# stefanopini/simple-HRNet

Hardware: AMD Instinct MI355X
Metric: person-crops/sec HRNet-W48 384x288 (model forward + heat-map decode) (higher is better)
Workload: dtype bf16; 1 GPU; HRNet-W48 384x288, batch=256 random crops per GPU, bf16 MFMA (BASELINE configs[2]); global_batch=256, micro_batch=256, lanes_per_gpu=1, parallelism=dp1 (crop sharding, RCCL all-gather of keypoints), weights=random-init seeded (synth_state_dict seed 0), BN stats randomised, engine_switches=

## Files before the change

### simple-hrnet_amd/csrc/conv3x3_lds.inc

```
typedef __attribute__((ext_vector_type(8))) __bf16 bf16x8;
typedef __attribute__((ext_vector_type(8))) short s16x8;
typedef __attribute__((ext_vector_type(4))) short s16x4;
typedef __attribute__((ext_vector_type(4))) float f32x4;
#define GLOBAL_AS __attribute__((address_space(1)))
typedef const GLOBAL_AS unsigned short *gcu16;
typedef GLOBAL_AS unsigned short *gu16;

__device__ __forceinline__ float relu1(float x) {
    float r;
    asm("v_max_f32 %0, 0, %1" : "=v"(r) : "v"(x));
    return r;
}

__device__ __forceinline__ void glds16(const GLOBAL_AS void *gsrc, char *lds_wave_base) {
    __builtin_amdgcn_global_load_lds(gsrc,
                                     (__attribute__((address_space(3))) void *)lds_wave_base, 16, 0, 0);
}

template <int KS_, int NRB_, int DT_ = DT_BF16>
struct C3Cfg {
    static constexpr int KS = KS_, NRB = NRB_;
    static constexpr int DT = DT_;
    static constexpr int PARTS = KS == 48 ? 2 : 1;
    static constexpr int CPP = KS == 48 ? 7 : 9;
// ... 435 lines not shown
            pk[i][2 * j + 1] = ok ? hi : 0u;
        }
    }
    asm volatile("s_waitcnt lgkmcnt(0)" ::: "memory");
    __builtin_amdgcn_s_barrier();
#pragma unroll
    for (int i = 0; i < NF; ++i) {
        const int yr = (i == NF - 1 ? row_last : row_first + i * 16) + li;
        const unsigned ya = lds0 + 2 * BBF_W + yr * ROWB + g * 24;
#pragma unroll
        for (int v = 0; v < 3; ++v)
            asm volatile("ds_write_b64 %0, %1 offset:%2" ::"v"(ya), "v"(u32x2{pk[i][2 * v], pk[i][2 * v + 1]}), "i"(v * 8) : "memory");
    }
    asm volatile("s_waitcnt lgkmcnt(0)" ::: "memory");
    __builtin_amdgcn_s_barrier();
}

template <int DT>
__device__ __forceinline__ void bbf_run(const Conv3Problem &p, const int mt0, const int tiles_this_block, const int nb, char *smem) {
    constexpr int KS = 48, NRB = 3, ROWB = 96, NCH = 14, BM = 512, MR = 4, NT = 512;
    typedef __attribute__((ext_vector_type(2))) unsigned u32x2;
    typedef __attribute__((ext_vector_type(4))) unsigned u32x4;
    const int tid = threadIdx.x, lane = tid & 63;
    const int wave = __builtin_amdgcn_readfirstlane(tid >> 6);
    const int li = lane & 15, g = lane >> 4;
    const int m = nb * p.hpwp;
    const int mtiles = (m + BM - 1) / BM;
    int ntile = mtiles - mt0;
    if (ntile > tiles_this_block) ntile = tiles_this_block;
    if (ntile <= 0) return;
    const int halo = p.wp + 1;
    const int xrows = BM + 4 * halo, yrows = BM + 2 * halo;
    const int xunits = xrows * 6;
    const int nfr = (yrows + 15) >> 4, base = nfr >> 3, extra = nfr & 7;
    const int cnt = base + (wave < extra ? 1 : 0);
    const int f0 = wave * base + (wave < extra ? wave : extra);
    const int row_first = f0 * 16;
    int row_last = (f0 + cnt - 1) * 16;
    if (row_last > yrows - 16) row_last = yrows - 16;
    const gcu16 in = (gcu16)p.in;
    const gu16 out = (gu16)p.out;
    const unsigned lds0 = (unsigned)(size_t)(__attribute__((address_space(3))) char *)smem;
    char *const xy = smem + 2 * BBF_W;

    int xoff[NCH];
#pragma unroll
    for (int c = 0; c < NCH; ++c) {
        int k0 = 32 * c + 8 * g;
        if (k0 >= 9 * KS) k0 = 0;
        const int tap = k0 / KS, ci = k0 - tap * KS;
        const int dh = tap / 3, dw = tap - 3 * dh;
        xoff[c] = (dh * p.wp + dw) * ROWB + (ci >> 3) * 16;
    }
    const int ch0 = g * 4 * NRB;
    const int bl = lane < KS ? lane : 0;
    const int bvec1 = __float_as_int(((const GLOBAL_AS float *)p.bias)[bl]);
    const int bvec2 = __float_as_int(((const GLOBAL_AS float *)p.bias2)[bl]);
    auto load_x = [&](int tt) {
        const long row0 = (long)(mt0 + tt) * BM - 2 * halo;
        const long lo = -(long)halo, hi = (long)m + halo + 511;
#pragma unroll
        for (int k = 0; k < BBF_XY / 16 / NT + 1; ++k) {
            if (k * NT + wave * 64 < xunits) {
                int u = k * NT + tid;
                asm volatile("" : "+v"(u));
                if (u >= xunits) u = xunits - 1;
                const int r = (int)(((unsigned)u * 43691u) >> 18);
                const int q8 = u - r * 6;
                long gr = row0 + r;
                gr = gr < lo ? lo : (gr > hi ? hi : gr);
                glds16((const GLOBAL_AS char *)(in + gr * KS + q8 * 8), xy + (k * NT + wave * 64) * 16);
            }
        }
    };
    constexpr int NXP = BBF_XY / 16 / NT + 1, NXR = 8;
    u32x4 xpre[NXR];
    const int r0u = (int)(((unsigned)tid * 43691u) >> 18), q0u = tid - r0u * 6;
    auto x_src = [&](int tt, int k) {
        const int row0 = (mt0 + tt) * BM - 2 * halo;
        int r = r0u, q8 = q0u;
        asm volatile("" : "+v"(r), "+v"(q8));
        r += 85 * k + (2 * k) / 6, q8 += (2 * k) % 6;
        if (q8 >= 6) q8 -= 6, ++r;
        if (r >= xrows) r = xrows - 1, q8 = 5;
        int gr = row0 + r;
        const int lo = -halo, hi = m + halo + 511;
        gr = gr < lo ? lo : (gr > hi ? hi : gr);
        return in + ((long)gr * KS + q8 * 8);
    };
    auto fetch_x = [&](int tt) {
#pragma unroll
        for (int k = 0; k < NXR; ++k) xpre[k] = *(const GLOBAL_AS u32x4 *)x_src(tt, k);
#pragma unroll
        for (int k = NXR; k < NXP; ++k)
            if (k * NT + wave * 64 < xunits) glds16((const GLOBAL_AS char *)x_src(tt, k), xy + (k * NT + wave * 64) * 16);
    };
    auto store_x = [&]() {
        const unsigned a0 = lds0 + 2 * BBF_W + tid * 16;
        asm volatile("s_waitcnt vmcnt(0)" ::: "memory");
#pragma unroll
        for (int k = 0; k < NXR; ++k)
            if (k * NT + wave * 64 < xunits)
                asm volatile("ds_write_b128 %0, %1 offset:%2" ::"v"(a0), "v"(xpre[k]), "i"(k * NT * 16) : "memory");
    };
    {
        const GLOBAL_AS char *w1 = (const GLOBAL_AS char *)p.w, *w2 = (const GLOBAL_AS char *)p.w2;
#pragma unroll
        for (int k = 0; k < (BBF_W / 16 + NT - 1) / NT; ++k) {
            const int u0 = k * NT + wave * 64;
            if (u0 < BBF_W / 16) {
                glds16(w1 + (size_t)(u0 + lane) * 16, smem + u0 * 16);
                glds16(w2 + (size_t)(u0 + lane) * 16, smem + BBF_W + u0 * 16);
            }
        }
        load_x(0);
    }
#ifdef HRN_C3_TIMING
    long long t_w = 0, t_c1 = 0, t_c1p = 0, t_c2 = 0, t_post = 0, t_epi = 0;
    C3_T(t_begin);
#endif
    for (int tt = 0; tt < ntile; ++tt) {
        C3_T(tA);
        if (tt == 0) asm volatile("s_waitcnt vmcnt(0)" ::: "memory");
        asm volatile("s_waitcnt lgkmcnt(0)" ::: "memory");
        __builtin_amdgcn_s_barrier();
        const long p0 = (long)(mt0 + tt) * BM;
        C3_T(tB);
        long long tC = 0;
        u32x2 rpre[MR][3];
        const unsigned res_a = lds0 + 2 * BBF_W + (wave * 16 * MR + li + 2 * halo) * ROWB + g * 24;
        if (cnt == 6)
            bbf_conv1<6, DT>(p, xoff, bvec1, lds0, row_first, row_last, p0 - halo, m, lane, res_a, rpre, tC);
        else if (cnt == 5)
            bbf_conv1<5, DT>(p, xoff, bvec1, lds0, row_first, row_last, p0 - halo, m, lane, res_a, rpre, tC);
        else
            bbf_conv1<4, DT>(p, xoff, bvec1, lds0, row_first, row_last, p0 - halo, m, lane, res_a, rpre, tC);
        C3_T(tD);
        if (tt + 1 < ntile) fetch_x(tt + 1);
        unsigned okbits2 = 0;
#pragma unroll
        for (int i = 0; i < MR; ++i) {
            const int q = (int)p0 + wave * 16 * MR + i * 16 + li;
            const int n_img = (int)(((unsigned long long)(unsigned)q * p.magic_hpwp) >> p.shift_hpwp);
            const int rem = q - n_img * p.hpwp;
            const int ho = (int)(((unsigned long long)(unsigned)rem * p.magic_wp) >> p.shift_wp);
            const int wo = rem - ho * p.wp;
            okbits2 |= ((q < m) && (ho < p.h) && (wo < p.wd)) ? 1u << i : 0u;
        }
        __builtin_amdgcn_sched_barrier(0);
        f32x4 acc[MR][NRB];
        {
            float bias2[4 * NRB];
#pragma unroll
            for (int c = 0; c < 4 * NRB; ++c) bias2[c] = __int_as_float(__builtin_amdgcn_ds_bpermute((ch0 + c) * 4, bvec2));
#pragma unroll
            for (int i = 0; i < MR; ++i)
#pragma unroll
                for (int j = 0; j < NRB; ++j) acc[i][j] = f32x4{bias2[j * 4], bias2[j * 4 + 1], bias2[j * 4 + 2], bias2[j * 4 + 3]};
        }
        {
            s16x8 wf[2][NRB], xf[2][MR];
            const unsigned wl_a = lds0 + BBF_W + lane * 16;
            unsigned sl_a = lds0 + 2 * BBF_W + (wave * 16 * MR + li) * ROWB;
            asm volatile("" : "+v"(sl_a));
#define BBF_READ2(SET, C)                                                                                         \
    {                                                                                                             \
        _Pragma("unroll") for (int j = 0; j < NRB; ++j)                                                           \
            asm volatile("ds_read_b128 %0, %1 offset:%2" : "=v"(wf[SET][j]) : "v"(wl_a), "i"(((C)*NRB + j) * 1024)); \
        const unsigned xa = sl_a + xoff[C];                                                                        \
        _Pragma("unroll") for (int i = 0; i < MR; ++i)                                                            \
            asm volatile("ds_read_b128 %0, %1 offset:%2" : "=v"(xf[SET][i]) : "v"(xa), "i"(i * 16 * ROWB));       \
    }
            BBF_READ2(0, 0)
#pragma unroll
            for (int c = 0; c < NCH; ++c) {
                const int cur = c & 1, nxt = cur ^ 1;
                if (c + 1 < NCH) {
                    BBF_READ2(nxt, c + 1)
                    asm volatile("s_waitcnt lgkmcnt(%0)" ::"i"(NRB + MR) : "memory");
                } else {
                    asm volatile("s_waitcnt lgkmcnt(0)" ::: "memory");
                }
                __builtin_amdgcn_sched_barrier(0);
#pragma unroll
                for (int i = 0; i < MR; ++i)
#pragma unroll
                    for (int j = 0; j < NRB; ++j)
                        acc[i][j] = H16<DT>::mma(wf[cur][j], xf[cur][i], acc[i][j]);
                __builtin_amdgcn_sched_barrier(0);
            }
#undef BBF_READ2
        }
        C3_T(tE);
        __builtin_amdgcn_s_barrier();
        if (tt + 1 < ntile) store_x();
        __builtin_amdgcn_sched_barrier(0);
        C3_T(tF);
#pragma unroll
        for (int i = 0; i < MR; ++i) {
            const int q = (int)p0 + wave * 16 * MR + i * 16 + li;
            const bool ok = (okbits2 >> i) & 1u;
            const size_t o = (size_t)q * KS + ch0;
            unsigned pk[2 * NRB];
#pragma unroll
            for (int j = 0; j < NRB; ++j) {
                const unsigned r01 = rpre[i][j][0], r23 = rpre[i][j][1];
                float v0 = acc[i][j][0] + H16<DT>::lo(r01);
                float v1 = acc[i][j][1] + H16<DT>::hi(r01);
                float v2 = acc[i][j][2] + H16<DT>::lo(r23);
                float v3 = acc[i][j][3] + H16<DT>::hi(r23);
                if (p.relu) v0 = relu1(v0), v1 = relu1(v1), v2 = relu1(v2), v3 = relu1(v3);
                const unsigned lo = H16<DT>::pk(v0, v1), hi = H16<DT>::pk(v2, v3);
                pk[2 * j] = ok ? lo : 0u;
                pk[2 * j + 1] = ok ? hi : 0u;
            }
            *(GLOBAL_AS u32x4 *)(out + o) = u32x4{pk[0], pk[1], pk[2], pk[3]};
            *(GLOBAL_AS u32x2 *)(out + o + 8) = u32x2{pk[4], pk[5]};
        }
#ifdef HRN_C3_TIMING
        C3_T(tG);
        t_w += tB - tA, t_c1 += tC - tB, t_c1p += tD - tC, t_c2 += tE - tD, t_post += tF - tE, t_epi += tG - tF;
#endif
    }
#ifdef HRN_C3_TIMING
    if (lane == 0 && g_c3_timing) {
        C3_T(t_end);
        long long *o = g_c3_timing + ((size_t)blockIdx.x * 8 + wave) * 8;
        o[0] = t_w, o[1] = t_c1, o[2] = t_c1p, o[3] = t_c2, o[4] = t_end - t_begin, o[5] = ntile, o[6] = 100 + cnt,
        o[7] = t_post | (t_epi << 32);
    }
#endif
}

#include "conv3x3_n96.inc"

template <int KS, int NRB, int DT>
__global__ __launch_bounds__(512, 2) void conv3x3_lds_kernel(const Conv3Problem *__restrict__ probs,
                                                             const int2 *__restrict__ blockmap, const int nb) {
    extern __shared__ __attribute__((aligned(16))) char smem[];
    using CFG = C3Cfg<KS, NRB, DT>;
#ifdef HRN_Q_TIMING
    struct Stamp {
        long long t0;
        __device__ Stamp() : t0((long long)__builtin_amdgcn_s_memrealtime()) {}
        __device__ ~Stamp() {
            if (g_q_timing && threadIdx.x == 0) {
                unsigned hw, xcc;
                asm volatile("s_getreg_b32 %0, hwreg(HW_REG_HW_ID)\n\ts_getreg_b32 %1, hwreg(HW_REG_XCC_ID)" : "=s"(hw), "=s"(xcc));
                const int seq = g_q_seq;
                long long *o = g_q_timing + ((size_t)(seq & (kQSlots - 1)) * kQBlocks + (blockIdx.x < kQBlocks ? blockIdx.x : kQBlocks - 1)) * 4;
                o[0] = t0, o[1] = (long long)gridDim.x | ((long long)seq << 32), o[2] = (long long)__builtin_amdgcn_s_memrealtime();
                o[3] = (long long)(((xcc & 15u) << 16) | (hw & 0xff00u));
            }
        }
    } stamp_;
#endif
    const int2 bm = blockmap[blockIdx.x];
    const Conv3Problem p = probs[bm.x & 0xff];
    const int nt = (bm.x >> 8) & 0xff, tiles = bm.x >> 16;
    const int mt0 = bm.y & 0x1fffffff;
    if constexpr (KS == 48 && NRB == 3) {
        if (bm.y & (1 << 29)) {
            bbf_run<DT>(p, mt0, tiles, nb, smem);
            return;
        }
        if (p.n96) {
            if (p.compact) {
                if (bm.y >> 30)
                    c3n_run<1, true, DT>(p, nt, mt0, tiles, nb, smem);
                else
                    c3n_run<4, true, DT>(p, nt, mt0, tiles, nb, smem);
                return;
            }
            if (bm.y >> 30)
                c3n_run<1, false, DT>(p, nt, mt0, tiles, nb, smem);
            else if (p.bm == 512)
                c3n_run<4, false, DT>(p, nt, mt0, tiles, nb, smem);
            else
                c3n_run<3, false, DT>(p, nt, mt0, tiles, nb, smem);
            return;
        }
    }
    if (bm.y >> 30) {
        conv3_run<CFG, 1>(p, nt, mt0, tiles, nb, smem);
    } else if constexpr (NRB == 4) {
        conv3_run<CFG, 3>(p, nt, mt0, tiles, nb, smem);
    } else {
        if (p.bm == 512)
            conv3_run<CFG, 4>(p, nt, mt0, tiles, nb, smem);
        else
            conv3_run<CFG, 3>(p, nt, mt0, tiles, nb, smem);
    }
}

template <int KS, int NRB, int DT>
static hipError_t launch_c3(const Conv3Problem *probs_dev, const int2 *blockmap_dev, int nblocks, int nb, hipStream_t s) {
// ... 27 lines not shown
```

### simple-hrnet_amd/csrc/ctx_memory.inc

```
    bool hip_ok(hipError_t e, const char *what) {
        if (e == hipSuccess) return true;
        err = std::string(what) + ": " + hipGetErrorString(e);
        return false;
    }

    bool allocate() {
        workspace_bytes = 0;
        for (auto &b : buffers) workspace_bytes += (int64_t)b.bytes;
        const int64_t small_crops = std::min<int64_t>(max_batch, (191 + head_slabs) / head_slabs);
        const int64_t part = std::max((int64_t)max_batch * joints * head_slabs, small_crops * joints * head_slabs_small);
        workspace_bytes += part * 8;
        if (plan_only) {
            fill_problems();
            index_s2groups();
            blob = (char *)calloc(1, (size_t)blob_bytes);
            return blob != nullptr;
        }
        if (!hip_ok(hipSetDevice(device), "hipSetDevice")) return false;
        for (auto &b : buffers) {
            if (!hip_ok(hipMalloc((void **)&b.dev, b.bytes), "hipMalloc(activation)")) return false;
            if (!hip_ok(hipMemset(b.dev, 0, b.bytes), "hipMemset(activation)")) return false;
        }
        if (!hip_ok(hipMalloc((void **)&blob, (size_t)blob_bytes), "hipMalloc(weights)")) return false;
        if (!hip_ok(hipMemset(blob, 0, (size_t)blob_bytes), "hipMemset(weights)")) return false;
// ... 18 lines not shown
    int group_blocks(const Conv3Group &g, int nb, std::vector<int2> *out, bool reverse, bool all_short = false,
                     std::vector<int> *tile_px_out = nullptr) const {
        struct Ent {
            double key;
            int2 v;
            int bm;
        };
        std::vector<Ent> ents;
        long one_per_block = 0;
        for (int ci : g.conv_idx) {
            const ConvOp &cv = convs[ci];
            if (skipped(cv, nb)) continue;
            const Tensor &to = tensors[cv.out_t];
            const int bmn = fused_now(cv, nb) ? 512 : conv3x3_lds_bm(cv.ks, cv.nr, to.wp);
            one_per_block += (long)((m_pixels(cv, to, nb) + bmn - 1) / bmn) * cv.ntiles;
        }
        const bool small = small_tiles && one_per_block < small_below;
        long small_blocks = 0;
        for (int ci : g.conv_idx) {
            const ConvOp &cv = convs[ci];
            if (skipped(cv, nb)) continue;
            small_blocks += (long)((m_pixels(cv, tensors[cv.out_t], nb) + 127) / 128) * cv.ntiles;
        }
        const bool keep_short_full = small && small_keep_above > 0 && small_blocks > small_keep_above;
        auto short_conv = [&](const ConvOp &cv) { return cv.ks != 16 && !cv.n96 && (cv.ks == 48 ? 2 : 1) * cv.slices <= 2; };
        auto small_conv = [&](const ConvOp &cv) {
            if (cv.ks == 16 && f32_small_slices > 0 && cv.slices >= f32_small_slices) return true;
            return small && !(keep_short_full && short_conv(cv));
        };
        auto tile_px = [&](const ConvOp &cv, const Tensor &to) {
            return fused_now(cv, nb) ? 512 : small_conv(cv) ? 128 : conv3x3_lds_bm(cv.ks, cv.nr, to.wp);
        };
        auto tiles_per_block = [&](const ConvOp &cv, int div) {
            return std::max(1, conv3_tiles_per_block(cv) / (fused_now(cv, nb) ? bbf_tpb_div : 1) / div);
        };
        auto count_blocks = [&](int div) {
            long total = 0;
            for (int ci : g.conv_idx) {
                const ConvOp &cv = convs[ci];
                if (skipped(cv, nb)) continue;
                const Tensor &to = tensors[cv.out_t];
                const int bm = tile_px(cv, to);
                const int mtiles = (int)((m_pixels(cv, to, nb) + bm - 1) / bm);
                const int tpb = tiles_per_block(cv, div);
                total += (long)((mtiles + tpb - 1) / tpb) * cv.ntiles;
            }
            return total;
        };
        int div = 1;
        while (div < 64 && count_blocks(div) < 512) div *= 2;
        int lf = all_short ? 1 : (int)std::min<long>(long_factor, count_blocks(div) / 768);
        if (lf < 1) lf = 1;
        for (size_t k = 0; k < g.conv_idx.size(); ++k) {
            const ConvOp &cv = convs[g.conv_idx[k]];
            if (skipped(cv, nb)) continue;
            const Tensor &to = tensors[cv.out_t];
            const int bm = tile_px(cv, to);
            const bool fused = fused_now(cv, nb);
            const int prob = fused ? g.fused_prob[k] : (int)k;
            const int mtiles = (int)((m_pixels(cv, to, nb) + bm - 1) / bm);
            const int tpb_short = tiles_per_block(cv, div);
            const int tpb_long = tpb_short * lf;
            const int long_tiles = ((int)(mtiles * long_share) / (8 * tpb_long)) * (8 * tpb_long);
            for (int phase = 0; phase < 2; ++phase) {
                const int tpb = phase == 0 ? tpb_long : tpb_short;
                const int first = phase == 0 ? 0 : long_tiles;
                const int count = phase == 0 ? long_tiles : mtiles - long_tiles;
                if (count <= 0) continue;
                const int mgroups = (count + tpb - 1) / tpb;
                const int total = mgroups * cv.ntiles;
                int seq = 0;
                for (int round = 0; round * 8 < mgroups; ++round)
                    for (int nt = 0; nt < cv.ntiles; ++nt)
                        for (int x = 0; x < 8; ++x) {
                            const int mg = round * 8 + x;
                            if (mg >= mgroups) continue;
                            const int i = seq++;
                            int tiles = count - mg * tpb;
                            if (tiles > tpb) tiles = tpb;
                            double key = (i + 0.5) / total;
                            if (block_order == 1)
                                key = -(double)tiles * (fused         ? 28000.0
                                                        : cv.ks == 16 ? cv.slices * (double)bm * 36.0 + 2000.0
                                                        : cv.n96      ? cv.slices * 3.0 * (bm == 512 ? 3900.0 : 3000.0) + (bm == 512 ? 7000.0 : 5000.0)
                                                                 : cv.slices * 2.0 * (bm == 512 ? 4300.0 : 3500.0) + (bm == 512 ? 5000.0 : 3000.0)) +
                                      1e-3 * key;
                            int mt0 = first + mg * tpb;
                            if (reverse) mt0 = mtiles - mt0 - tiles;
                            ents.push_back({key, int2{prob | (nt << 8) | (tiles << 16), mt0 | (fused ? 1 << 29 : small_conv(cv) ? 1 << 30 : 0)}, bm});
                        }
            }
        }
        std::stable_sort(ents.begin(), ents.end(), [](const Ent &a, const Ent &b) { return a.key < b.key; });
        if (tile_px_out) {
            tile_px_out->resize(ents.size());
            for (size_t i = 0; i < ents.size(); ++i) (*tile_px_out)[i] = ents[i].bm;
        }
        if (out) {
            out->resize(ents.size());
            for (size_t i = 0; i < ents.size(); ++i) (*out)[i] = ents[i].v;
        }
        return (int)ents.size();
    }

    const Tensor &grid_of(const ConvOp &cv) const { return tensors[cv.up ? cv.in_t : cv.out_t]; }

    ConvArgs conv_args(const ConvOp &cv, int nb, bool rev) const {
        const Tensor &ti = tensors[cv.in_t], &to = grid_of(cv);
        ConvArgs a;
        a.in = row0(cv.in_t), a.out = row0(cv.out_t);
        a.w = blob + cv.w_off, a.bias = (const float *)(blob + cv.b_off);
        a.res = cv.res_t >= 0 ? row0(cv.res_t) : nullptr;
        a.cin = cv.cin, a.cout = cv.cout;
        a.in_wp = ti.wp, a.in_hpwp = ti.hpwp;
        a.out_h = to.h, a.out_w = to.w, a.out_wp = to.wp, a.out_hpwp = to.hpwp;
        a.m = nb * to.hpwp;
        a.ksize = cv.k, a.stride = cv.stride, a.relu = cv.relu, a.kchunks = cv.kchunks;
        a.rev = rev;
// ... 240 lines not shown
        probs_host.assign(nprob, Conv3Problem{});
        std::vector<Conv3Problem> &hp = probs_host;
        for (auto &g : groups) {
            g.max_wp = 0;
            for (size_t k = 0; k < g.conv_idx.size(); ++k) {
                const ConvOp &cv = convs[g.conv_idx[k]];
                const Tensor &to = tensors[cv.out_t];
                Conv3Problem &q = hp[g.prob_first + k];
                q.in = row0(cv.in_t), q.out = row0(cv.out_t);
                q.w = blob + cv.w_off, q.bias = (const float *)(blob + cv.b_off);
                q.res = cv.res_t >= 0 ? row0(cv.res_t) : nullptr;
                q.cin = cv.cin, q.cout = cv.cout, q.h = to.h, q.wd = to.w, q.wp = to.wp, q.hpwp = to.hpwp;
                q.relu = cv.relu, q.slices = cv.slices, q.ntiles = cv.ntiles;
                q.w2 = nullptr, q.bias2 = nullptr;
                q.n96 = cv.n96 ? 1 : 0;
                q.compact = cv.compact ? 1 : 0, q.hw = to.h * to.w;
                q.slab_rows = q.slab_rows_small = 0;
                if (cv.compact) {
                    fast_div(q.hw, &q.magic_hw, &q.shift_hw);
                    fast_div(to.w, &q.magic_w, &q.shift_w);
                    q.slab_rows = compact_slab_rows(to.h, to.w, 512, max_batch), q.slab_rows_small = compact_slab_rows(to.h, to.w, 128, max_batch);
                }
                q.tiles_per_block = conv3_tiles_per_block(cv);
                q.bm = conv3x3_lds_bm(cv.ks, cv.nr, to.wp);
                fast_div(to.hpwp, &q.magic_hpwp, &q.shift_hpwp);
                fast_div(to.wp, &q.magic_wp, &q.shift_wp);
                if (to.wp > g.max_wp) g.max_wp = to.wp;
                if (cv.fuse_with >= 0) {
                    const ConvOp &c2 = convs[cv.fuse_with];
                    Conv3Problem &f = hp[g.prob_first + g.fused_prob[k]];
                    f = q;
                    f.out = row0(c2.out_t), f.relu = c2.relu, f.res = nullptr;
                    f.w2 = blob + c2.w_off, f.bias2 = (const float *)(blob + c2.b_off);
                }
            }
        }
        return nprob;
    }

    bool setup_groups() {
        const size_t nprob = fill_problems();
        if (!nprob) return true;
        std::vector<Conv3Problem> &hp = probs_host;
        for (auto &g : groups) {
            g.map_capacity = 64 + 4 * (int64_t)std::max(small_below, 256) + 1024;
            for (int ci : g.conv_idx) {
                const ConvOp &cv = convs[ci];
                const Tensor &to = tensors[cv.out_t];
                const int bm = f32_small_slices > 0 ? 128 : conv3x3_lds_bm(cv.ks, cv.nr, to.wp);
                g.map_capacity += (int64_t)((max_batch * to.hpwp + bm - 1) / bm) * cv.ntiles;
            }
            for (MapSlot &sl : g.slot) {
                if (!alloc_slot(sl, g.map_capacity, 0)) return false;
                workspace_bytes += g.map_capacity * (int64_t)sizeof(int2);
            }
        }
        if (!hip_ok(hipMalloc((void **)&probs_dev, nprob * sizeof(Conv3Problem)), "hipMalloc(problems)")) return false;
        return hip_ok(hipMemcpy(probs_dev, hp.data(), nprob * sizeof(Conv3Problem), hipMemcpyHostToDevice),
                      "hipMemcpy(problems)");
    }

    void free_all() {
        if (plan_only) {
            free(blob);
        } else {
            (void)hipSetDevice(device);
// ... 39 lines not shown
```

### simple-hrnet_amd/csrc/hrnet_mi355.cpp

```cpp
#include "../../include/hrnet_mi355.h"

#include <hip/hip_runtime.h>

#include <algorithm>
#include <cmath>
#include <cstdio>
#include <cstdlib>
#include <cstring>
#include <map>
#include <memory>
#include <string>
#include <vector>

#include "kernels.h"

namespace {
#include "ctx_types.h"
}

namespace {
thread_local std::string g_env_seen;
const char *env_sw(const char *name) {
    const char *v = hrn_env(name);
    if (v) {
// ... 27 lines not shown
        int conv3, conv1, ds;
        int conv2 = -1;
    };
    std::vector<Chain> chains;
    std::vector<TapPoint> taps;
    Conv3Problem *probs_dev = nullptr;
    std::vector<Op> ops;
    int stem_out_t = -1, head_in_t = -1;
    int64_t stem_w_off = 0, stem_b_off = 0, stem_wp_off = 0, head_w_off = 0, head_b_off = 0, head_wp_off = 0;

    int64_t blob_bytes = 0;
    char *blob = nullptr;
    bool weights_loaded = false;

    bool disable_lds = env_sw("HRN_DISABLE_LDS") != nullptr;
    bool disable_group = env_sw("HRN_DISABLE_GROUP") != nullptr;
    bool disable_dgroup = env_sw("HRN_DISABLE_DGROUP") != nullptr;
    bool disable_chain = env_sw("HRN_DISABLE_CHAIN") != nullptr;
    bool small_tiles = env_sw("HRN_SMALL_TILES") ? atoi(env_sw("HRN_SMALL_TILES")) != 0 : true;
    int small_below = env_sw("HRN_SMALL_BELOW") ? atoi(env_sw("HRN_SMALL_BELOW")) : 384;
    int small_keep_above = env_sw("HRN_SMALL_KEEP") ? atoi(env_sw("HRN_SMALL_KEEP")) : 300;
    bool disable_chain_ds = env_sw("HRN_DISABLE_CHAIN_DS") != nullptr;
    int pre_mode = env_sw("HRN_PRE_MODE") ? atoi(env_sw("HRN_PRE_MODE")) : 1;
    int chain_blocks = env_sw("HRN_CHAIN_BLOCKS") ? atoi(env_sw("HRN_CHAIN_BLOCKS")) : 512;
    bool disable_chain3 = env_sw("HRN_DISABLE_CHAIN3") != nullptr;
    bool direct_wlds = !(env_sw("HRN_DIRECT_WLDS") && atoi(env_sw("HRN_DIRECT_WLDS")) == 0);
    bool direct_xlds = !(env_sw("HRN_DIRECT_XLDS") && atoi(env_sw("HRN_DIRECT_XLDS")) == 0);
    bool conv_xl(const ConvOp &cv) const {
        return direct_xlds && direct_wlds && is16() && cv.k == 3 && cv.stride == 2 && cv.cin % 32 == 0 && !cv.up && cv.res_t < 0 && cv.nr == 6 &&
               cv.kchunks >= 4;
    }
    bool disable_bbf = env_sw("HRN_BBF") && atoi(env_sw("HRN_BBF")) == 0;
    int bbf_tpb_div = env_sw("HRN_BBF_TPB_DIV") ? std::max(1, atoi(env_sw("HRN_BBF_TPB_DIV"))) : 3;
    int bbf_min_tiles = env_sw("HRN_BBF_MIN_TILES") ? atoi(env_sw("HRN_BBF_MIN_TILES")) : 1100;
    int dgroup_nr_mode = env_sw("HRN_DGROUP_NR") ? atoi(env_sw("HRN_DGROUP_NR")) : 1;
    bool disable_lds32 = env_sw("HRN_DISABLE_LDS32") != nullptr;
    bool disable_n96 = env_sw("HRN_DISABLE_N96") != nullptr;
    bool disable_fgroup = env_sw("HRN_DISABLE_FGROUP") != nullptr;
    bool disable_f32lds = env_sw("HRN_DISABLE_F32LDS") != nullptr;
    int f32_small_slices = env_sw("HRN_F32_SMALL_SLICES") ? atoi(env_sw("HRN_F32_SMALL_SLICES")) : 0;
    std::vector<Conv3Problem> probs_host;
    bool disable_compact = env_sw("HRN_DISABLE_COMPACT") != nullptr;
    double compact_min_pad = env_sw("HRN_COMPACT_MIN_PAD") ? atof(env_sw("HRN_COMPACT_MIN_PAD")) : 0.08;
    bool disable_s2 = env_sw("HRN_DISABLE_S2") != nullptr;
    int s2_min_tiles = env_sw("HRN_S2_MIN_TILES") ? atoi(env_sw("HRN_S2_MIN_TILES")) : 256;
    int s2_target_blocks = env_sw("HRN_S2_BLOCKS") ? std::max(1, atoi(env_sw("HRN_S2_BLOCKS"))) : 256;
    bool disable_stem_mfma = env_sw("HRN_DISABLE_STEM_MFMA") != nullptr;
    bool disable_stem_fuse = env_sw("HRN_DISABLE_STEM_FUSE") != nullptr;
    bool stem_fuse = false;
    int stem_conv2_op = -1;
    S2Group stemf;
    bool disable_head_mfma = env_sw("HRN_DISABLE_HEAD_MFMA") != nullptr;
    bool direct_nr6 = env_sw("HRN_DIRECT_NR6") ? atoi(env_sw("HRN_DIRECT_NR6")) != 0 : true;
    int half_stages_per_block = env_sw("HRN_HALF_STAGES") ? atoi(env_sw("HRN_HALF_STAGES")) : 8;
    bool alternate = env_sw("HRN_ALTERNATE") ? atoi(env_sw("HRN_ALTERNATE")) != 0 : true;
    int block_order = env_sw("HRN_BLOCK_ORDER") ? atoi(env_sw("HRN_BLOCK_ORDER")) : 1;
    int long_factor = env_sw("HRN_LONG_FACTOR") ? atoi(env_sw("HRN_LONG_FACTOR")) : 4;
    double long_share = env_sw("HRN_LONG_SHARE") ? atof(env_sw("HRN_LONG_SHARE")) : 0.85;
    int head_slabs = 1, head_slab_px = 1024;
    static constexpr int kHeadSlabPxSmall = 256;
    int head_slabs_small = 1;
    int head_px_for(int nb) const { return (long)nb * head_slabs >= 192 ? head_slab_px : kHeadSlabPxSmall; }
    int head_slabs_for(int nb) const { return (long)nb * head_slabs >= 192 ? head_slabs : head_slabs_small; }
    float *part_val = nullptr;
    int *part_idx = nullptr;
    unsigned char *pre_tmp = nullptr;
// ... 645 lines not shown
```

### simple-hrnet_amd/csrc/kernels.h

```cpp
#pragma once
#include <hip/hip_runtime.h>
#include <stdint.h>

#include <atomic>
#include <cstdlib>
#include <cstring>

namespace hrn {

inline hipError_t set_dynamic_lds(const void *func, int bytes, std::atomic<unsigned long long> &done) {
    int dev = 0;
    hipError_t e = hipGetDevice(&dev);
    if (e != hipSuccess) return e;
    const unsigned long long bit = 1ull << (dev & 63);
    if (done.load(std::memory_order_acquire) & bit) return hipSuccess;
    e = hipFuncSetAttribute(func, hipFuncAttributeMaxDynamicSharedMemorySize, bytes);
    if (e == hipSuccess) done.fetch_or(bit, std::memory_order_release);
    return e;
}

inline const char *hrn_env(const char *name) {
    static const bool debug = [] {
        const char *v = getenv("HRN_DEBUG_ENV");
        return v && *v && strcmp(v, "0") != 0;
// ... 10 lines not shown
    const float *bias;
    const void *res;
    int cin, cout;
    int in_wp, in_hpwp;
    int out_h, out_w, out_wp, out_hpwp;
    int m;
    int ksize, stride, relu;
    int kchunks;
    int rev;
    int pre_mode;
    int wlds;
    int xlds;
    int up, up_a, up_b, up_wp, up_hpwp;
    int taps[4];
};

struct Conv3Problem {
    const void *in;
    void *out;
    const void *w;
    const float *bias;
    const void *res;
    int cin, cout;
    int h, wd, wp, hpwp;
    int relu;
    int slices;
    int ntiles;
    int tiles_per_block;
    int bm;
    unsigned magic_hpwp, magic_wp;
    int shift_hpwp, shift_wp;
    const void *w2;
    const float *bias2;
    int n96;
    int compact, hw;
    unsigned magic_hw, magic_w;
    int shift_hw, shift_w;
    int slab_rows, slab_rows_small;
};
int conv3x3_n96_ch64();
int conv3x3_lds_bbf_ok(int wp);
int conv3x3_n96_max_rows();
int conv3x3_lds_bm(int ks, int nrb, int wp);
int conv3x3_f32_bm(int wp);
hipError_t launch_conv3x3_f32(const Conv3Problem *probs_dev, const void *blockmap_dev, int nblocks, int nb, int nrb, hipStream_t s);

constexpr int kS2SlabBytes = 79872;
constexpr int s2_frags_per_part(int cin) { return cin == 48 ? 3 : 2; }
constexpr int s2_subslot_bytes(int cin) { return cin % 48 == 0 ? 96 : 32; }
constexpr int s2_region_bytes(int cin) { return kS2SlabBytes / (cin * 2 / s2_subslot_bytes(cin)) / 1024 * 1024; }
constexpr int s2_slot_capacity(int cin) { return s2_region_bytes(cin) / s2_subslot_bytes(cin); }
constexpr int s2_pair_pad(int wop) { return (8 - (3 * wop) % 8) % 8; }
constexpr int s2_pair_pitch(int wop) { return 4 * wop + s2_pair_pad(wop); }
constexpr int kS2MaxParts = 8;
struct S2Part {
    const void *w;
    const float *bias;
    void *out;
    int cout, ch0;
    int relu, pad_;
};
struct S2Problem {
    const void *in;
    int cin;
    int in_wp, in_hpwp;
    int ho, wo, wop, out_hpwp;
// ... 171 lines not shown
```

### simple-hrnet_amd/csrc/conv3x3_lds.hip

```cpp
#include "kernels.h"
#include "dt16.h"

namespace hrn {

#include "conv3x3_lds.inc"

#ifdef HRN_C3_TIMING
extern "C" int hrn_debug_c3_timing(long long *host_out, int max_blocks) {
    static long long *buf = nullptr;
    if (!buf) {
        if (hipMalloc((void **)&buf, (size_t)max_blocks * 512) != hipSuccess) return -1;
        (void)hipMemset(buf, 0, (size_t)max_blocks * 512);
        (void)hipMemcpyToSymbol(HIP_SYMBOL(g_c3_timing), &buf, sizeof(buf));
        return 0;
    }
    (void)hipDeviceSynchronize();
    (void)hipMemcpy(host_out, buf, (size_t)max_blocks * 512, hipMemcpyDeviceToHost);
    return 1;
}
#endif

#ifdef HRN_Q_TIMING
extern "C" int hrn_debug_q_timing(long long *host_out) {
    static long long *buf = nullptr;
    const size_t bytes = (size_t)kQSlots * kQBlocks * 4 * sizeof(long long);
    if (!buf) {
        if (hipMalloc((void **)&buf, bytes) != hipSuccess) return -1;
        (void)hipMemset(buf, 0, bytes);
        (void)hipMemcpyToSymbol(HIP_SYMBOL(g_q_timing), &buf, sizeof(buf));
        return 0;
    }
    (void)hipDeviceSynchronize();
    (void)hipMemcpy(host_out, buf, bytes, hipMemcpyDeviceToHost);
    return 1;
}
#endif

int conv3x3_n96_ch64() { return N96_CH64; }
int conv3x3_n96_max_rows() { return N96_MAXROWS; }

int conv3x3_lds_bbf_ok(int wp) { return (512 + 4 * (wp + 1)) * 6 <= BBF_XY / 16; }

int conv3x3_lds_bm(int ks, int nrb, int wp) {
    if (ks == 16) return conv3x3_f32_bm(wp);
    if (ks == 32 && nrb == 6) {
        auto fits = [&](int bm) { return (bm + 2 * wp + 2 + 15) / 16 * 16 <= N96_MAXROWS; };
        return fits(512) ? 512 : fits(384) ? 384 : 0;
    }
    const int maxrows = ks == 48 ? C3Cfg<48, 3>::MAXROWS : C3Cfg<32, 4>::MAXROWS;
    if (nrb != 4 && 512 + 2 * wp + 2 <= maxrows) return 512;
    if (384 + 2 * wp + 2 <= maxrows) return 384;
    return 0;
}

hipError_t launch_conv3x3_lds(const Conv3Problem *probs_dev, const void *blockmap_dev, int nblocks, int nb, int ks,
                              int nrb, hipStream_t s) {
    if (nblocks > 0 && ks == 16) return launch_conv3x3_f32(probs_dev, blockmap_dev, nblocks, nb, nrb, s);
    return launch_conv3x3_lds_t<DT_BF16>(probs_dev, blockmap_dev, nblocks, nb, ks, nrb, s);
}

}
```

Measured before the change: 11060 crops/s.

## Add ring-buffered producer/consumer fused basic-block conv kernel for 48-channel branch

Adds a new fused basic-block path (bbr_run) in which four waves compute the first 3x3 conv into a 4-band LDS ring while the other four waves consume it for the second conv plus residual, streaming input bands through a 7-band X ring with async global-to-LDS loads. Weights stay in registers for the whole block and each stage is software-pipelined, with one barrier per band. The aim is to replace the previous fused form with a steady-state pipeline that reuses LDS bands instead of recomputing halos per tile, at the cost of wave-role imbalance and a new tiles-per-block heuristic. It is enabled by default and can be switched off with HRN_BBF_FORM.

```diff
diff --git a/simple-hrnet_amd/csrc/conv3x3_lds.inc b/simple-hrnet_amd/csrc/conv3x3_lds.inc
--- a/simple-hrnet_amd/csrc/conv3x3_lds.inc
+++ b/simple-hrnet_amd/csrc/conv3x3_lds.inc
@@ -691,6 +691,243 @@
 #endif
 }
 
+constexpr int BBR_BANDB = 128 * 96;
+constexpr int BBR_YLEN = 4 * BBR_BANDB;
+constexpr int BBR_XLEN = 7 * BBR_BANDB;
+constexpr int BBR_LDS = BBR_YLEN + BBR_XLEN;
+static_assert(BBR_LDS <= BBF_LDS, "LDS budget");
+static_assert(BBR_YLEN + 16 < 65536, "the residual reads address the X ring through the 16-bit ds offset");
+
+__device__ __forceinline__ unsigned bbr_wrap(unsigned a, unsigned len) {
+    return __builtin_elementwise_min(a, a - len);
+}
+
+template <int DT, int RING, int RLEN>
+__device__ __forceinline__ void bbr_loop(const s16x8 (&wreg)[42], f32x4 (&acc)[2][3], unsigned a0, unsigned a1, const unsigned D,
+                                         const unsigned e4, const unsigned e13, const unsigned lds0) {
+    constexpr int NRB = 3, NCH = 14, NF = 2;
+    asm volatile("" : "+v"(a0), "+v"(a1));
+    s16x8 xf[2][NF];
+#define BBR_READ(SET, C)                                                                                                      \
+    {                                                                                                                         \
+        const unsigned so = 64u * (C) + ((C) >= 9 ? 2u * D : (C) >= 5 ? D : 0u);                                               \
+        const unsigned ev = (C) == 4 ? e4 : (C) == 13 ? e13 : 0u;                                                             \
+        const unsigned x0 = bbr_wrap(a0 + ev + so, RLEN) + lds0, x1 = bbr_wrap(a1 + ev + so, RLEN) + lds0;                    \
+        asm volatile("ds_read_b128 %0, %1 offset:%2" : "=v"(xf[SET][0]) : "v"(x0), "i"(RING));                               \
+        asm volatile("ds_read_b128 %0, %1 offset:%2" : "=v"(xf[SET][1]) : "v"(x1), "i"(RING));                               \
+    }
+    BBR_READ(0, 0)
+#pragma unroll
+    for (int c = 0; c < NCH; ++c) {
+        const int cur = c & 1, nxt = cur ^ 1;
+        if (c + 1 < NCH) {
+            BBR_READ(nxt, c + 1)
+            asm volatile("s_waitcnt lgkmcnt(%0)" ::"i"(NF) : "memory");
+        } else {
+            asm volatile("s_waitcnt lgkmcnt(0)" ::: "memory");
+        }
+        __builtin_amdgcn_sched_barrier(0);
+#pragma unroll
+        for (int f = 0; f < NF; ++f)
+#pragma unroll
+            for (int j = 0; j < NRB; ++j)
+                acc[f][j] = H16<DT>::mma(wreg[c * NRB + j], xf[cur][f], acc[f][j]);
+        __builtin_amdgcn_sched_barrier(0);
+    }
+#undef BBR_READ
+}
+
+template <int DT>
+__device__ __forceinline__ void bbr_run(const Conv3Problem &p, const int mt0, const int tiles_this_block, const int nb, char *smem) {
+    constexpr int KS = 48, NRB = 3, ROWB = 96, NCH = 14, BM = 512, NF = 2;
+    typedef __attribute__((ext_vector_type(2))) unsigned u32x2;
+    typedef __attribute__((ext_vector_type(4))) unsigned u32x4;
+    const int tid = threadIdx.x, lane = tid & 63;
+    const int wave = __builtin_amdgcn_readfirstlane(tid >> 6);
+    const int role = wave >> 2, wr = wave & 3;
+    const int li = lane & 15, g = lane >> 4;
+    const int m = nb * p.hpwp;
+    const int mtiles = (m + BM - 1) / BM;
+    int ntile = mtiles - mt0;
+    if (ntile > tiles_this_block) ntile = tiles_this_block;
+    if (ntile <= 0) return;
+    const int halo = p.wp + 1;
+    const int NB = 4 * ntile, NS = NB + 4;
+    const long P0 = (long)mt0 * BM;
+    const gcu16 in = (gcu16)p.in;
+    const gu16 out = (gu16)p.out;
+    const unsigned lds0 = (unsigned)(size_t)(__attribute__((address_space(3))) char *)smem;
+
+    const unsigned D = (unsigned)(p.wp - 3) * ROWB;
+    const unsigned e4 = g >= 2 ? D : 0u;
+    const unsigned e13 = g >= 2 ? 0u - (832u + 2u * D + 16u * g) : 0u;
+    const int ch0 = g * 4 * NRB;
+    const int bl = lane < KS ? lane : 0;
+    const int bvec = __float_as_int(((const GLOBAL_AS float *)(role ? p.bias2 : p.bias))[bl]);
+    s16x8 wreg[NCH * NRB];
+    {
+        const GLOBAL_AS char *w = (const GLOBAL_AS char *)(role ? p.w2 : p.w) + lane * 16;
+#pragma unroll
+        for (int k = 0; k < NCH * NRB; ++k) wreg[k] = *(const GLOBAL_AS s16x8 *)(w + k * 1024);
+    }
+    const int xlo = -halo, xhi = m + halo + 511;
+    auto load_xband = [&](int i) {
+        char *const dst = smem + BBR_YLEN + (i % 7) * BBR_BANDB;
+        const int row0 = (int)P0 - 256 + 128 * i;
+        int ln = lane;
+        asm volatile("" : "+v"(ln));
+#pragma unroll
+        for (int k = 0; k < 3; ++k) {
+            const int piece = wr + 4 * k;
+            const int u = piece * 64 + ln;
+            const int r = (int)(((unsigned)u * 43691u) >> 18);
+            const int q8 = u - r * 6;
+            int gr = row0 + r;
+            gr = gr < xlo ? xlo : (gr > xhi ? xhi : gr);
+            glds16((const GLOBAL_AS char *)(in + ((long)gr * KS + q8 * 8)), dst + piece * 1024);
+        }
+    };
+    const unsigned rlen = role ? BBR_YLEN : BBR_XLEN;
+    const int lrow = 32 * wr + li;
+    unsigned ra[NF];
+#pragma unroll
+    for (int f = 0; f < NF; ++f) {
+        const int r0 = role ? (128 - 384 - halo + lrow + 16 * f + 512) : (128 - halo + lrow + 16 * f);
+        ra[f] = (unsigned)r0 * ROWB + 16 * g;
+    }
+    f32x4 acc[NF][NRB];
+
+#ifdef HRN_C3_TIMING
+    long long t_wait = 0, t_loop = 0, t_tail = 0;
+    C3_T(t_begin);
+#endif
+    if (role == 0) {
+#pragma unroll
+        for (int i = 0; i < 4; ++i) load_xband(i);
+        asm volatile("s_waitcnt vmcnt(3)" ::: "memory");
+    }
+    __builtin_amdgcn_s_barrier();
+    for (int s = 0; s < NS; ++s) {
+        C3_T(tA);
+        if (role == 1 && s >= 4) {
+            const int k = s - 4;
+            u32x2 rpre[NF][3];
+#pragma unroll
+            for (int f = 0; f < NF; ++f) {
+                const unsigned xr = (unsigned)(((k + 2) % 7) * 128 + lrow + 16 * f) * ROWB + g * 24;
+#pragma unroll
+                for (int v = 0; v < 3; ++v)
+                    asm volatile("ds_read_b64 %0, %1 offset:%2" : "=v"(rpre[f][v]) : "v"(lds0 + xr), "i"(BBR_YLEN + v * 8));
+            }
+            unsigned okbits = 0;
+#pragma unroll
+            for (int f = 0; f < NF; ++f) {
+                const int q = (int)P0 + 128 * k + lrow + 16 * f;
+                const int n_img = (int)(((unsigned long long)(unsigned)q * p.magic_hpwp) >> p.shift_hpwp);
+                const int rem = q - n_img * p.hpwp;
+                const int ho = (int)(((unsigned long long)(unsigned)rem * p.magic_wp) >> p.shift_wp);
+                const int wo = rem - ho * p.wp;
+                okbits |= ((q < m) && (ho < p.h) && (wo < p.wd)) ? 1u << f : 0u;
+            }
+            asm volatile("s_waitcnt lgkmcnt(0)" ::: "memory");
+#pragma unroll
+            for (int f = 0; f < NF; ++f) {
+                const int q = (int)P0 + 128 * k + lrow + 16 * f;
+                const bool ok = (okbits >> f) & 1u;
+                const size_t o = (size_t)q * KS + ch0;
+                unsigned pk[2 * NRB];
+#pragma unroll
+                for (int j = 0; j < NRB; ++j) {
+                    const unsigned r01 = rpre[f][j][0], r23 = rpre[f][j][1];
+                    float v0 = acc[f][j][0] + H16<DT>::lo(r01);
+                    float v1 = acc[f][j][1] + H16<DT>::hi(r01);
+                    float v2 = acc[f][j][2] + H16<DT>::lo(r23);
+                    float v3 = acc[f][j][3] + H16<DT>::hi(r23);
+                    if (p.relu) v0 = relu1(v0), v1 = relu1(v1), v2 = relu1(v2), v3 = relu1(v3);
+                    const unsigned lo = H16<DT>::pk(v0, v1), hi = H16<DT>::pk(v2, v3);
+                    pk[2 * j] = ok ? lo : 0u;
+                    pk[2 * j + 1] = ok ? hi : 0u;
+                }
+                *(GLOBAL_AS u32x4 *)(out + o) = u32x4{pk[0], pk[1], pk[2], pk[3]};
+                *(GLOBAL_AS u32x2 *)(out + o + 8) = u32x2{pk[4], pk[5]};
+            }
+        }
+        C3_T(tB);
+        const bool active = role == 0 ? s < NB + 2 : (s >= 3 && s < NB + 3);
+        if (active) {
+            {
+                float bias[4 * NRB];
+                int cb = ch0 * 4;
+                asm volatile("" : "+v"(cb));
+#pragma unroll
+                for (int c = 0; c < 4 * NRB; ++c) bias[c] = __int_as_float(__builtin_amdgcn_ds_bpermute(cb + c * 4, bvec));
+#pragma unroll
+                for (int f = 0; f < NF; ++f)
+#pragma unroll
+                    for (int j = 0; j < NRB; ++j) acc[f][j] = f32x4{bias[j * 4], bias[j * 4 + 1], bias[j * 4 + 2], bias[j * 4 + 3]};
+            }
+            if (role == 0)
+                bbr_loop<DT, BBR_YLEN, BBR_XLEN>(wreg, acc, ra[0], ra[1], D, e4, e13, lds0);
+            else
+                bbr_loop<DT, 0, BBR_YLEN>(wreg, acc, ra[0], ra[1], D, e4, e13, lds0);
+        }
+        C3_T(tC);
+        if (role == 0) {
+            if (active) {
+                unsigned okbits = 0;
+#pragma unroll
+                for (int f = 0; f < NF; ++f) {
+                    const int q = (int)P0 - 128 + 128 * s + lrow + 16 * f;
+                    const unsigned uq = (unsigned)q;
+                    const int n_img = (int)(((unsigned long long)uq * p.magic_hpwp) >> p.shift_hpwp);
+                    const int rem = (int)uq - n_img * p.hpwp;
+                    const int ho = (int)(((unsigned long long)(unsigned)rem * p.magic_wp) >> p.shift_wp);
+                    const int wo = rem - ho * p.wp;
+                    okbits |= (q >= 0 && q < m && ho < p.h && wo < p.wd) ? 1u << f : 0u;
+                }
+#pragma unroll
+                for (int f = 0; f < NF; ++f) {
+                    const bool ok = (okbits >> f) & 1u;
+                    unsigned pk[2 * NRB];
+#pragma unroll
+                    for (int j = 0; j < NRB; ++j) {
+                        const unsigned lo = H16<DT>::pk(relu1(acc[f][j][0]), relu1(acc[f][j][1]));
+                        const unsigned hi = H16<DT>::pk(relu1(acc[f][j][2]), relu1(acc[f][j][3]));
+                        pk[2 * j] = ok ? lo : 0u;
+                        pk[2 * j + 1] = ok ? hi : 0u;
+                    }
+                    const unsigned ya = lds0 + (unsigned)((s & 3) * 128 + lrow + 16 * f) * ROWB + g * 24;
+#pragma unroll
+                    for (int v = 0; v < 3; ++v)
+                        asm volatile("ds_write_b64 %0, %1 offset:%2" ::"v"(ya), "v"(u32x2{pk[2 * v], pk[2 * v + 1]}), "i"(v * 8) : "memory");
+                }
+            }
+            if (s + 4 < NB + 4) {
+                load_xband(s + 4);
+                asm volatile("s_waitcnt vmcnt(3) lgkmcnt(0)" ::: "memory");
+            } else {
+                asm volatile("s_waitcnt vmcnt(0) lgkmcnt(0)" ::: "memory");
+            }
+        }
+        C3_T(tD);
+        __builtin_amdgcn_s_barrier();
+#ifdef HRN_C3_TIMING
+        C3_T(tE);
+        if (role == 0) t_loop += tC - tB, t_tail += tD - tC, t_wait += tE - tD + tB - tA;
+        else t_tail += tB - tA, t_loop += tC - tB, t_wait += tE - tC;
+#endif
+#pragma unroll
+        for (int f = 0; f < NF; ++f) ra[f] = bbr_wrap(ra[f] + BBR_BANDB, rlen);
+    }
+#ifdef HRN_C3_TIMING
+    if (lane == 0 && g_c3_timing) {
+        C3_T(t_end);
+        long long *o = g_c3_timing + ((size_t)blockIdx.x * 8 + wave) * 8;
+        o[0] = t_wait, o[1] = t_loop, o[2] = t_tail, o[3] = 0, o[4] = t_end - t_begin, o[5] = NS, o[6] = 200 + role, o[7] = ntile;
+    }
+#endif
+}
+
 #include "conv3x3_n96.inc"
 
 template <int KS, int NRB, int DT>
@@ -720,7 +957,10 @@
     const int mt0 = bm.y & 0x1fffffff;
     if constexpr (KS == 48 && NRB == 3) {
         if (bm.y & (1 << 29)) {
-            bbf_run<DT>(p, mt0, tiles, nb, smem);
+            if (p.bbr)
+                bbr_run<DT>(p, mt0, tiles, nb, smem);
+            else
+                bbf_run<DT>(p, mt0, tiles, nb, smem);
             return;
         }
         if (p.n96) {
diff --git a/simple-hrnet_amd/csrc/ctx_memory.inc b/simple-hrnet_amd/csrc/ctx_memory.inc
--- a/simple-hrnet_amd/csrc/ctx_memory.inc
+++ b/simple-hrnet_amd/csrc/ctx_memory.inc
@@ -74,6 +74,7 @@
             return fused_now(cv, nb) ? 512 : small_conv(cv) ? 128 : conv3x3_lds_bm(cv.ks, cv.nr, to.wp);
         };
         auto tiles_per_block = [&](const ConvOp &cv, int div) {
+            if (fused_now(cv, nb) && bbf_form) return std::max(1, bbr_tiles / div);
             return std::max(1, conv3_tiles_per_block(cv) / (fused_now(cv, nb) ? bbf_tpb_div : 1) / div);
         };
         auto count_blocks = [&](int div) {
@@ -122,7 +123,7 @@
                             if (tiles > tpb) tiles = tpb;
                             double key = (i + 0.5) / total;
                             if (block_order == 1)
-                                key = -(double)tiles * (fused         ? 28000.0
+                                key = -(double)tiles * (fused         ? (bbf_form ? 12500.0 + 25000.0 / tiles : 28000.0)
                                                         : cv.ks == 16 ? cv.slices * (double)bm * 36.0 + 2000.0
                                                         : cv.n96      ? cv.slices * 3.0 * (bm == 512 ? 3900.0 : 3000.0) + (bm == 512 ? 7000.0 : 5000.0)
                                                                  : cv.slices * 2.0 * (bm == 512 ? 4300.0 : 3500.0) + (bm == 512 ? 5000.0 : 3000.0)) +
@@ -432,6 +433,7 @@
                     f = q;
                     f.out = row0(c2.out_t), f.relu = c2.relu, f.res = nullptr;
                     f.w2 = blob + c2.w_off, f.bias2 = (const float *)(blob + c2.b_off);
+                    f.bbr = bbf_form;
                 }
             }
         }
diff --git a/simple-hrnet_amd/csrc/hrnet_mi355.cpp b/simple-hrnet_amd/csrc/hrnet_mi355.cpp
--- a/simple-hrnet_amd/csrc/hrnet_mi355.cpp
+++ b/simple-hrnet_amd/csrc/hrnet_mi355.cpp
@@ -83,6 +83,8 @@
     }
     bool disable_bbf = env_sw("HRN_BBF") && atoi(env_sw("HRN_BBF")) == 0;
     int bbf_tpb_div = env_sw("HRN_BBF_TPB_DIV") ? std::max(1, atoi(env_sw("HRN_BBF_TPB_DIV"))) : 3;
+    int bbf_form = env_sw("HRN_BBF_FORM") ? (atoi(env_sw("HRN_BBF_FORM")) != 0) : 1;
+    int bbr_tiles = env_sw("HRN_BBR_TILES") ? std::max(1, atoi(env_sw("HRN_BBR_TILES"))) : 4;
     int bbf_min_tiles = env_sw("HRN_BBF_MIN_TILES") ? atoi(env_sw("HRN_BBF_MIN_TILES")) : 1100;
     int dgroup_nr_mode = env_sw("HRN_DGROUP_NR") ? atoi(env_sw("HRN_DGROUP_NR")) : 1;
     bool disable_lds32 = env_sw("HRN_DISABLE_LDS32") != nullptr;
diff --git a/simple-hrnet_amd/csrc/kernels.h b/simple-hrnet_amd/csrc/kernels.h
--- a/simple-hrnet_amd/csrc/kernels.h
+++ b/simple-hrnet_amd/csrc/kernels.h
@@ -66,6 +66,7 @@
     int shift_hpwp, shift_wp;
     const void *w2;
     const float *bias2;
+    int bbr;
     int n96;
     int compact, hw;
     unsigned magic_hw, magic_w;
```

Measured after the change: 11120 crops/s (median of 6 runs). No clear change (+0.5%).

## Carry conv1 halo rows across consecutive tiles in fused basic-block kernel

Applied to the files above, without the earlier changes.

In the fused two-conv basic-block kernel, consecutive M-tiles processed by one block now reuse the overlapping halo rows of the intermediate conv1 output. Those rows are read from LDS into registers and written back at the start of the next tile's buffer, so later tiles fetch less input and recompute conv1 over fewer rows (fixed 4-fragment path). The block-ordering cost model is updated to charge a cheaper per-extra-tile slide cost, and the eligibility check now requires room for the carried rows. The cost is added LDS traffic and extra waits, plus more complex index bookkeeping that could introduce correctness errors at tile boundaries.

```diff
diff --git a/simple-hrnet_amd/csrc/conv3x3_lds.hip b/simple-hrnet_amd/csrc/conv3x3_lds.hip
--- a/simple-hrnet_amd/csrc/conv3x3_lds.hip
+++ b/simple-hrnet_amd/csrc/conv3x3_lds.hip
@@ -39,7 +39,10 @@
 int conv3x3_n96_ch64() { return N96_CH64; }
 int conv3x3_n96_max_rows() { return N96_MAXROWS; }
 
-int conv3x3_lds_bbf_ok(int wp) { return (512 + 4 * (wp + 1)) * 6 <= BBF_XY / 16; }
+int conv3x3_lds_bbf_ok(int wp) {
+    const int cunits = 2 * (wp + 1) * 6;
+    return (512 + 4 * (wp + 1)) * 6 <= BBF_XY / 16 && 3072 + cunits + (cunits + 63) / 64 * 64 <= BBF_XY / 16;
+}
 
 int conv3x3_lds_bm(int ks, int nrb, int wp) {
     if (ks == 16) return conv3x3_f32_bm(wp);
diff --git a/simple-hrnet_amd/csrc/conv3x3_lds.inc b/simple-hrnet_amd/csrc/conv3x3_lds.inc
--- a/simple-hrnet_amd/csrc/conv3x3_lds.inc
+++ b/simple-hrnet_amd/csrc/conv3x3_lds.inc
@@ -491,6 +491,7 @@
     const int halo = p.wp + 1;
     const int xrows = BM + 4 * halo, yrows = BM + 2 * halo;
     const int xunits = xrows * 6;
+    const int cunits = 2 * halo * 6;
     const int nfr = (yrows + 15) >> 4, base = nfr >> 3, extra = nfr & 7;
     const int cnt = base + (wave < extra ? 1 : 0);
     const int f0 = wave * base + (wave < extra ? wave : extra);
@@ -532,14 +533,15 @@
             }
         }
     };
-    constexpr int NXP = BBF_XY / 16 / NT + 1, NXR = 8;
+    constexpr int NXR = 6, NXP = NXR + 2;
     u32x4 xpre[NXR];
+    const int xu0 = cunits;
     const int r0u = (int)(((unsigned)tid * 43691u) >> 18), q0u = tid - r0u * 6;
     auto x_src = [&](int tt, int k) {
         const int row0 = (mt0 + tt) * BM - 2 * halo;
         int r = r0u, q8 = q0u;
         asm volatile("" : "+v"(r), "+v"(q8));
-        r += 85 * k + (2 * k) / 6, q8 += (2 * k) % 6;
+        r += 2 * halo + 85 * k + (2 * k) / 6, q8 += (2 * k) % 6;
         if (q8 >= 6) q8 -= 6, ++r;
         if (r >= xrows) r = xrows - 1, q8 = 5;
         int gr = row0 + r;
@@ -552,15 +554,21 @@
         for (int k = 0; k < NXR; ++k) xpre[k] = *(const GLOBAL_AS u32x4 *)x_src(tt, k);
 #pragma unroll
         for (int k = NXR; k < NXP; ++k)
-            if (k * NT + wave * 64 < xunits) glds16((const GLOBAL_AS char *)x_src(tt, k), xy + (k * NT + wave * 64) * 16);
+            if (xu0 + k * NT + wave * 64 < xunits) glds16((const GLOBAL_AS char *)x_src(tt, k), xy + (xu0 + k * NT + wave * 64) * 16);
     };
     auto store_x = [&]() {
-        const unsigned a0 = lds0 + 2 * BBF_W + tid * 16;
+        const unsigned a0 = lds0 + 2 * BBF_W + (xu0 + tid) * 16;
         asm volatile("s_waitcnt vmcnt(0)" ::: "memory");
 #pragma unroll
         for (int k = 0; k < NXR; ++k)
-            if (k * NT + wave * 64 < xunits)
-                asm volatile("ds_write_b128 %0, %1 offset:%2" ::"v"(a0), "v"(xpre[k]), "i"(k * NT * 16) : "memory");
+            asm volatile("ds_write_b128 %0, %1 offset:%2" ::"v"(a0), "v"(xpre[k]), "i"(k * NT * 16) : "memory");
+    };
+    u32x4 ycar[2];
+    const unsigned ca0 = lds0 + 2 * BBF_W + (tid < cunits ? tid : 0) * 16;
+    const unsigned ca1 = lds0 + 2 * BBF_W + (tid + NT < cunits ? tid + NT : 0) * 16;
+    auto store_carry = [&]() {
+        if (tid < cunits) asm volatile("ds_write_b128 %0, %1" ::"v"(ca0), "v"(ycar[0]) : "memory");
+        if (tid + NT < cunits) asm volatile("ds_write_b128 %0, %1" ::"v"(ca1), "v"(ycar[1]) : "memory");
     };
     {
         const GLOBAL_AS char *w1 = (const GLOBAL_AS char *)p.w, *w2 = (const GLOBAL_AS char *)p.w2;
@@ -588,14 +596,16 @@
         long long tC = 0;
         u32x2 rpre[MR][3];
         const unsigned res_a = lds0 + 2 * BBF_W + (wave * 16 * MR + li + 2 * halo) * ROWB + g * 24;
-        if (cnt == 6)
-            bbf_conv1<6, DT>(p, xoff, bvec1, lds0, row_first, row_last, p0 - halo, m, lane, res_a, rpre, tC);
-        else if (cnt == 5)
-            bbf_conv1<5, DT>(p, xoff, bvec1, lds0, row_first, row_last, p0 - halo, m, lane, res_a, rpre, tC);
+        const int rf = tt > 0 ? 2 * halo + wave * 64 : row_first, rl = tt > 0 ? rf + 48 : row_last;
+        if (tt == 0 && cnt == 6)
+            bbf_conv1<6, DT>(p, xoff, bvec1, lds0, rf, rl, p0 - halo, m, lane, res_a, rpre, tC);
+        else if (tt == 0 && cnt == 5)
+            bbf_conv1<5, DT>(p, xoff, bvec1, lds0, rf, rl, p0 - halo, m, lane, res_a, rpre, tC);
         else
-            bbf_conv1<4, DT>(p, xoff, bvec1, lds0, row_first, row_last, p0 - halo, m, lane, res_a, rpre, tC);
+            bbf_conv1<4, DT>(p, xoff, bvec1, lds0, rf, rl, p0 - halo, m, lane, res_a, rpre, tC);
         C3_T(tD);
-        if (tt + 1 < ntile) fetch_x(tt + 1);
+        const bool carry = tt + 1 < ntile;
+        if (carry) fetch_x(tt + 1);
         unsigned okbits2 = 0;
 #pragma unroll
         for (int i = 0; i < MR; ++i) {
@@ -639,6 +649,10 @@
                     asm volatile("s_waitcnt lgkmcnt(%0)" ::"i"(NRB + MR) : "memory");
                 } else {
                     asm volatile("s_waitcnt lgkmcnt(0)" ::: "memory");
+                    if (carry) {
+                        asm volatile("ds_read_b128 %0, %1 offset:%2" : "=v"(ycar[0]) : "v"(ca0), "i"(BM * ROWB) : "memory");
+                        asm volatile("ds_read_b128 %0, %1 offset:%2" : "=v"(ycar[1]) : "v"(ca1), "i"(BM * ROWB) : "memory");
+                    }
                 }
                 __builtin_amdgcn_sched_barrier(0);
 #pragma unroll
@@ -651,8 +665,12 @@
 #undef BBF_READ2
         }
         C3_T(tE);
+        asm volatile("s_waitcnt lgkmcnt(0)" ::: "memory");
         __builtin_amdgcn_s_barrier();
-        if (tt + 1 < ntile) store_x();
+        if (carry) {
+            store_carry();
+            store_x();
+        }
         __builtin_amdgcn_sched_barrier(0);
         C3_T(tF);
 #pragma unroll
diff --git a/simple-hrnet_amd/csrc/ctx_memory.inc b/simple-hrnet_amd/csrc/ctx_memory.inc
--- a/simple-hrnet_amd/csrc/ctx_memory.inc
+++ b/simple-hrnet_amd/csrc/ctx_memory.inc
@@ -122,10 +122,10 @@
                             if (tiles > tpb) tiles = tpb;
                             double key = (i + 0.5) / total;
                             if (block_order == 1)
-                                key = -(double)tiles * (fused         ? 28000.0
-                                                        : cv.ks == 16 ? cv.slices * (double)bm * 36.0 + 2000.0
+                                key = -(fused ? 28000.0 + (tiles - 1) * bbf_slide_cost
+                                        : (double)tiles * (cv.ks == 16 ? cv.slices * (double)bm * 36.0 + 2000.0
                                                         : cv.n96      ? cv.slices * 3.0 * (bm == 512 ? 3900.0 : 3000.0) + (bm == 512 ? 7000.0 : 5000.0)
-                                                                 : cv.slices * 2.0 * (bm == 512 ? 4300.0 : 3500.0) + (bm == 512 ? 5000.0 : 3000.0)) +
+                                                                 : cv.slices * 2.0 * (bm == 512 ? 4300.0 : 3500.0) + (bm == 512 ? 5000.0 : 3000.0))) +
                                       1e-3 * key;
                             int mt0 = first + mg * tpb;
                             if (reverse) mt0 = mtiles - mt0 - tiles;
diff --git a/simple-hrnet_amd/csrc/hrnet_mi355.cpp b/simple-hrnet_amd/csrc/hrnet_mi355.cpp
--- a/simple-hrnet_amd/csrc/hrnet_mi355.cpp
+++ b/simple-hrnet_amd/csrc/hrnet_mi355.cpp
@@ -83,6 +83,7 @@
     }
     bool disable_bbf = env_sw("HRN_BBF") && atoi(env_sw("HRN_BBF")) == 0;
     int bbf_tpb_div = env_sw("HRN_BBF_TPB_DIV") ? std::max(1, atoi(env_sw("HRN_BBF_TPB_DIV"))) : 3;
+    double bbf_slide_cost = env_sw("HRN_BBF_SLIDE_COST") ? atof(env_sw("HRN_BBF_SLIDE_COST")) : 24600.0;
     int bbf_min_tiles = env_sw("HRN_BBF_MIN_TILES") ? atoi(env_sw("HRN_BBF_MIN_TILES")) : 1100;
     int dgroup_nr_mode = env_sw("HRN_DGROUP_NR") ? atoi(env_sw("HRN_DGROUP_NR")) : 1;
     bool disable_lds32 = env_sw("HRN_DISABLE_LDS32") != nullptr;
```

After: 11410 crops/s before, 11640 crops/s after (median of 6 runs). 1.02x the previous value.
